# Ogeon/pyrite

Hardware: AMD Instinct MI355X
Metric: Msamples/sec (higher is better)
Workload: dtype f32; 1 GPU; C3: c3_mesh_in_box, 1920x1080, 1024 spp; bounces=8, light_samples=4, spectrum_samples=10, spectrum_bins=64, tile_size=32, triangles=819212, spheres=0, parallelism=one launch on one GPU, film_weight_check=ok

## Files before the change

### pyrite_amd/csrc/kernels.hip

```cpp
#ifndef PYRITE_KERNELS_HIP
#define PYRITE_KERNELS_HIP
#include <hip/hip_runtime.h>

#include <algorithm>
#include <cstdint>
#include <cstdlib>
#include <string>
#include <type_traits>

#include "device_scene.h"
#include "exact_math.h"

#ifdef PYR_WIDE_VM
#define PYR_VM_NUMBERS PYR_WIDE_NUMBER_REGISTERS
#define PYR_VM_VECTORS PYR_WIDE_VECTOR_REGISTERS
#define PYR_VM_RGBS PYR_WIDE_RGB_REGISTERS
#else
#define PYR_VM_NUMBERS PYR_MAX_NUMBER_REGISTERS
#define PYR_VM_VECTORS PYR_MAX_VECTOR_REGISTERS
#define PYR_VM_RGBS PYR_MAX_RGB_REGISTERS
#endif
static_assert((PYR_VM_NUMBERS & (PYR_VM_NUMBERS - 1)) == 0 && (PYR_VM_VECTORS & (PYR_VM_VECTORS - 1)) == 0 && (PYR_VM_RGBS & (PYR_VM_RGBS - 1)) == 0,
              "the interpreter masks register indices: its files are powers of two");

// ... 1153 lines not shown
            const float* from = reinterpret_cast<const float*>(src);
            if (COPY)
                for (uint32_t i = threadIdx.x; i < floats; i += BLOCK) dst[i] = from[i];
            float* at = dst;
            dst += floats;
            return at;
        };
        local.spectra = reinterpret_cast<const PyrSpectrum*>(stage(S.spectra, S.num_spectra * (uint32_t)(sizeof(PyrSpectrum) / sizeof(float))));
        local.spectrum_data = stage(S.spectrum_data, S.num_spectrum_floats);
        local.materials = reinterpret_cast<const PyrMaterial*>(stage(S.materials, S.num_materials * (uint32_t)(sizeof(PyrMaterial) / sizeof(float))));
        local.components = reinterpret_cast<const PyrComponent*>(stage(S.components, S.num_components * (uint32_t)(sizeof(PyrComponent) / sizeof(float))));
        local.programs = reinterpret_cast<const DevProgram*>(stage(S.programs, S.num_programs * (uint32_t)(sizeof(DevProgram) / sizeof(float))));
        local.lamps = reinterpret_cast<const DevLamp*>(stage(S.lamps, S.num_lamps * (uint32_t)(sizeof(DevLamp) / sizeof(float))));
        if (COPY) __syncthreads();
    }
    return local;
}

template <bool COMPANION_STATE = true>
DEV void start_sample(const RenderLaunch& L, uint32_t tile, uint64_t iteration, const TileArea& area, Path& p, Spectral& spec) {
    const uint32_t SS = L.spectrum_samples;
    p.rng = rng_seed(L.seed, tile, iteration);
    const float px = __fadd_rn(area.from_x, __fmul_rn(area.size_x, rng_f32(p.rng)));
    const float py = __fadd_rn(area.from_y, __fmul_rn(area.size_y, rng_f32(p.rng)));
    p.pixel = film_pixel(L, tile, px, py);
    {
        float focus_x = px / L.camera.view_plane * L.camera.focus_distance;
        float focus_y = py / L.camera.view_plane * L.camera.focus_distance;
        f3 target = mk(focus_x, -focus_y, -L.camera.focus_distance);
        f3 origin = mk(0, 0, 0), direction = target;
        if (L.camera.aperture > 0.0f) {
            float sqrt_r = sqrt32(L.camera.aperture * rng_f32(p.rng));
            float psi = PI_F * 2.0f * rng_f32(p.rng);
            origin = mk(sqrt_r * cos32(psi), sqrt_r * sin32(psi), 0.0f);
            direction = target - origin;
        }
        p.o = transform_point(L.camera.cam_to_world, origin);
        p.d = transform_vector(L.camera.cam_to_world, normalize(direction));
    }
    {
        float step_size = L.film.wl_width / (float)SS;
        float from = L.film.wl_start;
        for (uint32_t k = 0; k < SS; ++k) {
            float to = __fadd_rn(from, step_size);
            spec.wl(k) = rng_range_f32(p.rng, from, to);
            from = to;
        }
        uint32_t hero = rng_range_usize(p.rng, SS);
        p.wl = spec.wl(hero);
        spec.wl(hero) = spec.wl(SS - 1);
        if constexpr (COMPANION_STATE)
            for (uint32_t k = 0; k + 1 < SS; ++k) {
                spec.bright(k) = 0.0f;
                spec.refl(k) = 1.0f;
            }
    }
    p.bright = 0.0f;
    p.refl = 1.0f;
    p.use_additional = true;
    p.sample_light = true;
    p.events = 0;
    p.bounce = 0;
}

DEV bool locate_chunk(const RenderLaunch& L, uint32_t chunk, uint32_t lane, uint32_t& tile, uint64_t& iteration, TileArea& area) {
    const uint32_t k = chunk / L.chunks_per_tile, within = chunk - k * L.chunks_per_tile;
    tile = L.tile_begin + k * L.tile_stride;
    const uint32_t ty = tile / L.tiles_x, tx = tile - ty * L.tiles_x;
    const uint32_t sx = tx * L.tile_size, sy = ty * L.tile_size;
    const uint32_t w = min(L.film.width - sx, L.tile_size), h = min(L.film.height - sy, L.tile_size);
    const uint64_t area_px = (uint64_t)w * h, iterations = area_px * L.pixel_samples;
    iteration = (uint64_t)within * 64u + lane;
    if (iteration >= iterations) return false;
    iteration += area_px * L.sample_begin;
    area = to_view_area(sx, sy, w, h, L.film.width, L.film.height);
    return true;
}

struct SyncProf {
    unsigned long long section[8] = {0, 0, 0, 0, 0, 0, 0, 0}, last = 0;
};
#ifdef PYR_PHASE_PROFILE
__device__ unsigned long long g_phase_prof[16];
#define SLAP(sp, i)                                 \
    {                                               \
        const unsigned long long now_ = clock64();  \
        (sp).section[i] += now_ - (sp).last;        \
        (sp).last = now_;                           \
    }
#else
#define SLAP(sp, i)
#endif

constexpr int SYNC_PRIO_T = 3, SYNC_PRIO_N = 2, SYNC_PRIO_S = 1, SYNC_PRIO_E = 0;
#define SYNC_PRIO(x) __builtin_amdgcn_s_setprio(x)
template <bool COUNT>
DEV bool bounce_step(const DevScene& S, const RenderLaunch& L, const SceneView& view, Path& p, Spectral& spec, int* stack, Counters& cnt, SyncProf& sp) {
    const uint32_t n_add = L.spectrum_samples - 1;
    Hit hit;
    if (COUNT) cnt.extension_rays++;
    const f3 ray_o = p.o, ray_d = p.d;
    SYNC_PRIO(SYNC_PRIO_T);
    const bool found = traverse<COUNT, false>(S, view.nodes, view.prims, ray_o, ray_d, 0.0f, hit, stack, cnt);
    SYNC_PRIO(SYNC_PRIO_S);
    SLAP(sp, 1);
    if (!found) {
        uint32_t color = S.sky_program;
        if (p.sample_light) {
            for (uint32_t i = 0; i < S.num_lamps; ++i) {
                const DevLamp& l = S.lamps[i];
                if (l.kind == PYR_LAMP_DIRECTIONAL && dot(ld3(l.v), ray_d) >= l.width) {
                    color = l.color_program;
                    break;
                }
            }
        }
        const Prepared q_prog = prepare_program<false>(S, color);
        VmInput in{p.wl, -ray_d, ray_d};
        p.bright += eval_prepared<false>(S, q_prog, in) * 1.0f * p.refl;
        if (p.use_additional)
            for (uint32_t k = 0; k < n_add; ++k) {
                in.wavelength = spec.wl(k);
                spec.bright(k) += eval_prepared<false>(S, q_prog, in) * 1.0f * spec.refl(k);
            }
        return true;
    }
    if (COUNT) cnt.shaded_hits++;
    f3 position, normal;
    uint32_t material_id;
    surface_at(S, hit, ray_o, ray_d, position, normal, material_id);
    const PyrMaterial material = S.materials[material_id];
    const uint32_t pick = rng_choose(p.rng, material.num_components);
    const PyrComponent comp = S.components[material.first_component + pick];
    float component_probability = comp.selection_compensation;
    bool normal_dispersed = false;
    if (comp.probability_program >= 0) {
        VmInput pin{p.wl, normal, ray_d};
        component_probability = run_program<false>(S, (uint32_t)comp.probability_program, pin) * comp.selection_compensation;
        normal_dispersed = S.programs[comp.probability_program].reads_wavelength != 0;
    }

    if (comp.bsdf == PYR_BSDF_EMISSIVE) {
        if (p.sample_light) {
            p.use_additional = !normal_dispersed && p.use_additional;
            const Prepared q_prog = prepare_program<false>(S, comp.color_program);
            VmInput in{p.wl, normal, ray_d};
            p.bright += eval_prepared<false>(S, q_prog, in) * component_probability * p.refl;
            if (p.use_additional)
                for (uint32_t k = 0; k < n_add; ++k) {
                    in.wavelength = spec.wl(k);
                    spec.bright(k) += eval_prepared<false>(S, q_prog, in) * component_probability * spec.refl(k);
                }
        }
        return true;
    }

    f3 out_direction;
    float scatter_probability = 1.0f;
    bool dispersed = false, has_brdf = false;
    if (comp.bsdf == PYR_BSDF_DIFFUSE) {
        f3 n = dot(ray_d, normal) < 0.0f ? normal : -normal;
        out_direction = sample_hemisphere(p.rng, n);
        has_brdf = true;
    } else if (comp.bsdf == PYR_BSDF_MIRROR) {
        f3 n = dot(ray_d, normal) < 0.0f ? normal : -normal;
        float perp = dot(ray_d, n) * 2.0f;
// ... 112 lines not shown
        if (p.use_additional)
            for (uint32_t k = 0; k < n_add; ++k) spec.refl(k) *= brdf;
    }
    p.o = position;
    p.d = out_direction;
    SLAP(sp, 6);
    return false;
}

template <bool COUNT>
DEV void finish_path(const RenderLaunch& L, const Path& p, Spectral& spec, Counters& cnt) {
    expose_grain<COUNT>(L, p.pixel, p.wl, p.bright, cnt);
    if (p.use_additional)
        for (uint32_t k = 0; k + 1 < L.spectrum_samples; ++k) expose_grain<COUNT>(L, p.pixel, spec.wl(k), spec.bright(k), cnt);
}

typedef __attribute__((address_space(4))) const RenderLaunch* kernarg_launch_ptr;
constexpr size_t kLaunchKernargOffset = (sizeof(DevScene) + alignof(RenderLaunch) - 1) / alignof(RenderLaunch) * alignof(RenderLaunch);
typedef __attribute__((address_space(4))) const DevScene* kernarg_scene_ptr;
DEV const DevScene& scene_from_kernarg(const DevScene& ) {
    unsigned long long at = (unsigned long long)__builtin_amdgcn_kernarg_segment_ptr();
    asm volatile("" : "+s"(at));
    return *(const DevScene*)(kernarg_scene_ptr)at;
}
DEV const RenderLaunch& launch_from_kernarg(const RenderLaunch& ) {
    unsigned long long at = (unsigned long long)__builtin_amdgcn_kernarg_segment_ptr() + kLaunchKernargOffset;
    asm volatile("" : "+s"(at));
    return *(const RenderLaunch*)(kernarg_launch_ptr)at;
}

template <bool COUNT, bool LDS_SCENE, bool LDS_TABLES>
__global__ __launch_bounds__(BLOCK, 4) void render_kernel(DevScene S0, RenderLaunch L) {
    extern __shared__ float lds[];
    const uint32_t SS = L.spectrum_samples;
    Spectral spec{lds + threadIdx.x, SS};
    int* stack = reinterpret_cast<int*>(lds + 3 * SS * BLOCK) + threadIdx.x;
    Counters cnt{};
    const uint32_t lds_base_floats = (3 * SS + S0.stack_depth) * BLOCK;
    const SceneView view = stage_scene<LDS_SCENE>(S0, lds, lds_base_floats);
    const DevScene S = stage_tables<LDS_TABLES ? 1 : 0>(S0, lds, lds_base_floats + (LDS_SCENE ? (S0.num_nodes * 16 + S0.num_prims * 12) : 0));

    const uint32_t lane = threadIdx.x & 63u;
    const uint32_t waves_per_block = BLOCK / 64;
    const uint32_t wave = blockIdx.x * waves_per_block + (threadIdx.x >> 6);
    const uint32_t total_waves = gridDim.x * waves_per_block;

    SyncProf sp;
#ifdef PYR_PHASE_PROFILE
    sp.last = clock64();
#endif
    for (uint32_t chunk = L.chunk_begin + wave; chunk < L.chunk_end; chunk += total_waves) {
        uint32_t tile;
        uint64_t iteration;
        TileArea area;
        if (!locate_chunk(L, chunk, lane, tile, iteration, area)) continue;
        Path p{};
        start_sample(launch_from_kernarg(L), tile, iteration, area, p, spec);
        if (COUNT) cnt.samples++;
        SLAP(sp, 0);
        while (p.bounce < L.bounces) {
            const bool ended = bounce_step<COUNT>(S, launch_from_kernarg(L), view, p, spec, stack, cnt, sp);
            p.bounce++;
            if (ended) break;
        }
        SLAP(sp, 6);
        SYNC_PRIO(SYNC_PRIO_E);
        finish_path<COUNT>(launch_from_kernarg(L), p, spec, cnt);
        SLAP(sp, 7);
    }
#ifdef PYR_PHASE_PROFILE
    if (lane == 0)
        for (int i = 0; i < 8; ++i) atomicAdd(&g_phase_prof[i], sp.section[i]);
#endif
    flush_counters<COUNT>(cnt, L.counters);
}

#ifdef PYR_PHASE_PROFILE
#define PROF_DECL unsigned long long prof_c[4] = {0, 0, 0, 0}, prof_l[4] = {0, 0, 0, 0}, prof_n[4] = {0, 0, 0, 0}
#define PROF_BEGIN(ph, cond) const unsigned long long prof_t0_##ph = clock64(); prof_l[ph] += __popcll(ballot64(cond)); prof_n[ph]++
#define PROF_END(ph) prof_c[ph] += clock64() - prof_t0_##ph
#define PROF_LANES(ph, cond) prof_l[ph] += __popcll(ballot64(cond)); prof_n[ph]++
#define PROF_NOW() clock64()
#define PROF_EXTRA(idx, cycles) if ((threadIdx.x & 63u) == 0) atomicAdd(&g_phase_prof[idx], (unsigned long long)(cycles))
#define PROF_FLUSH()                                                                                  \
    if ((threadIdx.x & 63u) == 0)                                                                     \
        for (int i = 0; i < 4; ++i) {                                                                 \
            atomicAdd(&g_phase_prof[i], prof_c[i]);                                                   \
            atomicAdd(&g_phase_prof[4 + i], prof_l[i]);                                               \
            atomicAdd(&g_phase_prof[8 + i], prof_n[i]);                                               \
        }
#else
#define PROF_DECL
#define PROF_BEGIN(ph, cond)
#define PROF_END(ph)
#define PROF_LANES(ph, cond)
#define PROF_NOW() 0ull
#define PROF_EXTRA(idx, cycles)
#define PROF_FLUSH()
#endif

enum Stage : uint32_t { ST_NEW = 0, ST_TRAV = 1, ST_SHADE = 2, ST_NEE = 3, ST_EXPOSE = 4, ST_DONE = 5 };

struct Trav {
    f3 o, d, inv;
    uint32_t nx = 0, ny = 0, nz = 0;
    float limit, closest;
    int node, sp;
    uint32_t shape;
    float u, v;
    bool shadow, blocked;
};

DEV void trav_ray_signs(Trav& t) {
    t.nx = (__float_as_uint(t.d.x) >> 31) * 48u;
    t.ny = (__float_as_uint(t.d.y) >> 31) * 48u;
    t.nz = (__float_as_uint(t.d.z) >> 31) * 48u;
}
DEV float shadow_cutoff(float limit, float margin) { return __builtin_amdgcn_sqrtf(limit * margin + 1.0e-3f); }
DEV void trav_restart(Trav& t, float shadow_margin) {
    if (t.shadow) t.closest = shadow_cutoff(t.limit, shadow_margin);
    t.blocked = false;
    t.node = 0;
    t.sp = 0;
}

template <bool COUNT>
DEV bool trav_begin(const DevScene& S, Trav& t, f3 o, f3 d, bool shadow, float limit, Counters& cnt) {
    t.o = o;
    t.d = d;
    t.shadow = shadow;
    t.blocked = false;
    t.limit = shadow ? limit : -PYR_INF;
    t.closest = PYR_INF;
    t.shape = PYR_HIT_NONE;
    t.u = t.v = 0.0f;
    for (uint32_t i = 0; i < S.num_planes; ++i) {
        const float* pl = S.planes + 8 * i;
        float dist;
        f3 point;
        if (COUNT) cnt.plane_tests++;
        if (plane_test(ld3(pl), ld3(pl + 3), o, d, dist, point)) {
            if (shadow) {
                if (dist > DIST_EPSILON && dist * dist < limit) {
                    t.blocked = true;
                    return true;
                }
            } else if (dist > DIST_EPSILON && dist < t.closest) {
                t.closest = dist;
                t.shape = ((uint32_t)PYR_SHAPE_PLANE << 30) | i;
            }
        }
    }
    trav_restart(t, S.shadow_margin);
    return false;
}

typedef __attribute__((address_space(3))) int lds_int;
struct TravStack {
    lds_int* lds;
    int lds_entries;
    int* deep;
    DEV void push(int sp, int value) {
        if (sp < lds_entries)
            lds[sp * BLOCK] = value;
        else
            deep[sp - lds_entries] = value;
    }
    DEV int pop(int sp) const { return sp < lds_entries ? lds[sp * BLOCK] : deep[sp - lds_entries]; }
};

template <bool COUNT, bool SIGNED = false>
DEV void wide_node_children(const float4 lx, const float4 ly, const float4 lz, const float4 hx, const float4 hy, const float4 hz, const float4 ch, const Trav& t,
                            Counters& cnt, float (&e)[4], int (&c)[4]) {
    const f2v ix = {t.inv.x, t.inv.x}, iy = {t.inv.y, t.inv.y}, iz = {t.inv.z, t.inv.z};
    const float ox = -(t.o.x * t.inv.x), oy = -(t.o.y * t.inv.y), oz = -(t.o.z * t.inv.z);
    const f2v nox = {ox, ox}, noy = {oy, oy}, noz = {oz, oz};
    c[0] = __float_as_int(ch.x), c[1] = __float_as_int(ch.y), c[2] = __float_as_int(ch.z), c[3] = __float_as_int(ch.w);
    {
        const f2v alx = __builtin_elementwise_fma((f2v){lx.x, lx.y}, ix, nox), ahx = __builtin_elementwise_fma((f2v){hx.x, hx.y}, ix, nox);
        const f2v aly = __builtin_elementwise_fma((f2v){ly.x, ly.y}, iy, noy), ahy = __builtin_elementwise_fma((f2v){hy.x, hy.y}, iy, noy);
// ... 690 lines not shown
                    contribution(CONTRIB_ADD, l_color, deferred_probability, material_probability, true, ls_scale, p.use_additional && !l_dispersed, target_normal, t.d,
                                 ls_physical ? ls_tx : 0.0f, ls_physical ? ls_ty : 0.0f);
                } else {
                    const Prepared q_prog = prepare_program<INTERP>(S, l_color);
                    VmInput in{p.wl, target_normal, t.d, ls_physical ? ls_tx : 0.0f, ls_physical ? ls_ty : 0.0f};
                    p.bright += eval_prepared<INTERP>(S, q_prog, in) * l_probability * p.refl;
                    if (p.use_additional && !l_dispersed)
                        for (uint32_t k = 0; k < n_add; ++k) {
                            in.wavelength = spec.wl(k);
                            spec.bright(k) += eval_prepared<INTERP>(S, q_prog, in) * l_probability * spec.refl(k);
                        }
                }
            }
        }
        const DevLamp& lamp = S.lamps[nee_lamp];
        while (nee_i < L.light_samples) {
            const LampSample ls = lamp_sample<INTERP>(lamp, p.rng, b_position);
            nee_i++;
            const float cos_out = fmaxf(dot(b_nff(), ls.direction), 0.0f);
            if (!(cos_out > 0.0f)) continue;
            if (COUNT) cnt.shadow_rays++;
            const float limit = ls.sq_distance >= 0.0f ? ls.sq_distance - DIST_EPSILON : PYR_INF;
            ls_scale = ls.weight * nee_probability(S, L) * (2.0f * fabsf(dot(ls.direction, b_nff())));
            ls_physical = ls.physical;
            ls_material = ls.material;
            ls_color = ls.color;
            ls_normal = ls.normal;
            ls_tx = ls.tx, ls_ty = ls.ty;
            ls_pending = true;
            stage = trav_begin<COUNT>(S, t, b_position, ls.direction, true, limit, cnt) ? ST_NEE : ST_TRAV;
            break;
        }
        if (stage == ST_NEE && !ls_pending) finish_bounce(S, L, spec, cnt);
    }
};

DEV float lambda_eval(const DevScene& S, const DevProgram& p, float wavelength) {
    float num[PYR_MAX_NUMBER_REGISTERS];
    auto value = [&](const PyrOperand& o) -> float {
        if (o.kind == PYR_OPERAND_CONSTANT) return __uint_as_float(o.bits);
        if (o.kind == PYR_OPERAND_INPUT) return wavelength;
        return num[o.bits & (PYR_MAX_NUMBER_REGISTERS - 1)];
    };
    for (uint32_t k = 0; k < p.num_instrs; ++k) {
        const PyrInstr& ins = S.instrs[p.first_instr + k];
        float r = 0.0f;
        switch (ins.op) {
        case PYR_OP_NUMBER: r = __uint_as_float(ins.x.bits); break;
        case PYR_OP_SPECTRUM: r = spectrum_get(S, ins.a, value(ins.x)); break;
        case PYR_OP_BLACKBODY: {
            const float wl = value(ins.x), temp = value(ins.y);
            r = blackbody(wl, temp);
            break;
        }
        case PYR_OP_MIX: {
            const float amount = fmaxf(fminf(value(ins.x), 1.0f), 0.0f);
            const float l = num[ins.a & (PYR_MAX_NUMBER_REGISTERS - 1)], rr = num[ins.b & (PYR_MAX_NUMBER_REGISTERS - 1)];
            r = l * (1.0f - amount) + rr * amount;
            break;
        }
        case PYR_OP_BINARY: {
            const float l = num[ins.a & (PYR_MAX_NUMBER_REGISTERS - 1)], rr = num[ins.b & (PYR_MAX_NUMBER_REGISTERS - 1)];
            r = ins.operator_ == PYR_BIN_ADD ? l + rr : (ins.operator_ == PYR_BIN_SUB ? l - rr : (ins.operator_ == PYR_BIN_MUL ? l * rr : l / rr));
            break;
        }
        default: {
            const float v = value(ins.x), mn = value(ins.y), mx = value(ins.z);
            r = fmaxf(fminf(v, mx), mn);
            break;
        }
        }
        num[ins.output & (PYR_MAX_NUMBER_REGISTERS - 1)] = r;
    }
    return num[p.output_reg & (PYR_MAX_NUMBER_REGISTERS - 1)];
}

template <bool COUNT, bool RGB = false, bool TIMES = false>
DEV void replay_tapes(const DevScene& S, const RenderLaunch& L, bool exposing, uint32_t n_ops, uint32_t tape_column, const Path& p, const float* wl_rows,
                      uint32_t wl_column, uint32_t* wave_list, const uint32_t* prepared_lds, float* spectral_values, uint32_t n_spectral, bool eager, Counters& cnt) {
    const uint32_t lane = threadIdx.x & 63u;
    const unsigned long long mask = ballot64(exposing);
    const uint32_t n = (uint32_t)__popcll(mask);
    if (n == 0) return;
    uint32_t max_ops = exposing ? (n_ops < L.tape_max_ops ? n_ops : L.tape_max_ops) : 0u;
    const uint32_t my_ops = max_ops;
    for (int off = 32; off > 0; off >>= 1) max_ops = max(max_ops, (uint32_t)__shfl_xor((int)max_ops, off));
    const bool keeps = exposing && p.use_additional, lost = exposing && !p.use_additional;
    const bool longest = 3u * my_ops > 2u * max_ops, shortest = 3u * my_ops <= max_ops;
    const unsigned long long below = (1ull << lane) - 1ull;
    const unsigned long long k0 = ballot64(keeps && longest), k1 = ballot64(keeps && !longest && !shortest), k2 = ballot64(keeps && shortest);
    const unsigned long long l0 = ballot64(lost && longest), l1 = ballot64(lost && !longest && !shortest), l2 = ballot64(lost && shortest);
    const uint32_t n_full = (uint32_t)__builtin_popcountll(k0 | k1 | k2);
    if (exposing) {
        const unsigned long long mine = keeps ? (longest ? k0 : (shortest ? k2 : k1)) : (longest ? l0 : (shortest ? l2 : l1));
        uint32_t before = keeps ? 0u : n_full;
        before += (uint32_t)__builtin_popcountll(keeps ? ((longest ? 0ull : k0) | (shortest ? k1 : 0ull)) : ((longest ? 0ull : l0) | (shortest ? l1 : 0ull)));
        wave_list[before + (uint32_t)__builtin_popcountll(mine & below)] = lane;
    }
    __builtin_amdgcn_wave_barrier();
    const uint32_t SS = L.spectrum_samples, full_items = n_full * SS, items = full_items + (n - n_full);
    const unsigned long long past_the_end =
        eager ? ((unsigned long long)(kTapeOneSlot << TAPE_EAGER_SLOT_SHIFT) | ((unsigned long long)__float_as_uint(1.0f) << 32)) : 0ull;
#ifndef PYR_REPLAY_ROWS
#define PYR_REPLAY_ROWS 8
#endif
    constexpr uint32_t ROWS = PYR_REPLAY_ROWS;
    for (uint32_t base = 0; base < items; base += 64) {
        const uint32_t i = base + lane;
        const bool active = i < items;
        const bool full = i < full_items;
        const uint32_t rank = !active ? 0u : (full ? i / SS : n_full + (i - full_items)), k = !active ? 0u : (full ? i - rank * SS : SS - 1u);
        const uint32_t src = wave_list[rank];
        const uint32_t ops = (uint32_t)__shfl((int)n_ops, (int)src);
        uint32_t pass_ops = active ? (ops < L.tape_max_ops ? ops : L.tape_max_ops) : 0u;
        for (int off = 32; off > 0; off >>= 1) pass_ops = max(pass_ops, (uint32_t)__shfl_xor((int)pass_ops, off));
        const uint32_t pixel = (uint32_t)__shfl((int)p.pixel, (int)src);
        const float hero_wl = __shfl(p.wl, (int)src);
        const bool hero = k == SS - 1;
        const bool run = active;
        const uint32_t src_column = (uint32_t)__shfl((int)wl_column, (int)src);
        const float wl = hero ? hero_wl : wl_rows[k * BLOCK + src_column];
        float refl = 1.0f, bright = 0.0f, value = 0.0f;
        uint32_t value_of = 0xFFFFFFFFu;
        [[maybe_unused]] float rgb_sum = 0.0f;
        if (eager) {
            const uint32_t* slot_program = prepared_lds + 8 * L.tape_programs_lds;
            uint32_t grid_min = 0, grid_max = 0, grid_count = 0;
            uint32_t i0 = 0, i1 = 0;
            float mix = 0.0f;
            bool below = false, above = false;
            for (uint32_t slot = 0; slot < n_spectral; ++slot) {
                const uint32_t* e = prepared_lds + 8 * slot_program[slot];
                const uint32_t mode = e[0], format = e[2], count = e[6];
                const float c = __uint_as_float(e[1]);
                const float* data = S.spectrum_data + e[5];
                float v;
                if (RGB && mode == 0xFFu) {
                    v = lambda_eval(S, S.programs[slot_program[slot]], wl);
                } else if (format == PYR_SPECTRUM_ARRAY && count != 0u) {
                    if (e[3] != grid_min || e[4] != grid_max || count != grid_count) {
                        grid_min = e[3], grid_max = e[4], grid_count = count;
                        const float lo = __uint_as_float(grid_min), hi = __uint_as_float(grid_max);
                        below = wl <= lo, above = wl >= hi;
                        const float normalized = (wl - lo) / (hi - lo);
                        const float float_index = normalized * ((float)count - 1.0f);
                        const float min_float_index = truncf(float_index);
                        i0 = (below | above) ? 0u : (uint32_t)min_float_index;
                        i1 = (below | above) ? 0u : i0 + 1u;
                        mix = float_index - min_float_index;
                    }
                    const float inside = data[i0] * (1.0f - mix) + data[i1] * mix;
                    v = below ? data[0] : (above ? data[count - 1] : inside);
                } else {
                    PyrSpectrum sp;
                    sp.format = format, sp.min = __uint_as_float(e[3]), sp.max = __uint_as_float(e[4]), sp.offset = e[5], sp.count = count;
                    v = spectrum_eval(sp, data, wl);
                }
                spectral_values[tape_row(slot) * BLOCK] = (mode == FAST_SPECTRUM || mode == 0xFFu) ? v : v * c;
            }
            if (RGB && S.rgb_records != 0) {
                float resp[3] = {0.0f, 0.0f, 0.0f};
                const uint32_t count = S.rgb_count;
                if (count > 0) {
                    const float* d = S.rgb_basis;
                    if (wl <= S.rgb_min) {
                        for (int j = 0; j < 3; ++j) resp[j] = d[j];
                    } else if (wl >= S.rgb_max) {
                        for (int j = 0; j < 3; ++j) resp[j] = d[3 * (count - 1) + j];
                    } else {
                        const float normalized = (wl - S.rgb_min) / (S.rgb_max - S.rgb_min);
                        const float fi = normalized * ((float)count - 1.0f);
                        const float fmin_ = truncf(fi);
                        const uint32_t b0 = (uint32_t)fmin_;
                        const float bmix = fi - fmin_;
                        for (int j = 0; j < 3; ++j) resp[j] = d[3 * b0 + j] * (1.0f - bmix) + d[3 * (b0 + 1) + j] * bmix;
                    }
                }
                for (uint32_t j = 0; j < 3; ++j) spectral_values[(tape_rgb_row(n_spectral) + j) * BLOCK] = resp[j];
            }
        }
        for (uint32_t r0 = 0; r0 < pass_ops; r0 += ROWS) {
            unsigned long long rows[ROWS];
#pragma unroll
            for (uint32_t j = 0; j < ROWS; ++j) rows[j] = r0 + j < my_ops ? L.tape[tape_index(r0 + j, L.tape_lanes, tape_column)] : past_the_end;
            uint32_t words[ROWS];
            float factors[ROWS];
#pragma unroll
            for (uint32_t j = 0; j < ROWS; ++j) {
                words[j] = (uint32_t)__shfl((int)(uint32_t)rows[j], (int)src);
                factors[j] = __uint_as_float((uint32_t)__shfl((int)(uint32_t)(rows[j] >> 32), (int)src));
            }
            if (eager) {
                float values[ROWS];
#pragma unroll
                for (uint32_t j = 0; j < ROWS; ++j) values[j] = spectral_values[words[j] & TAPE_EAGER_SLOT_MASK];
                if (RGB && (TIMES ? S.micro_records : S.rgb_records) != 0) {
                    const uint32_t not_mine = hero ? 0u : TAPE_HERO_ONLY;
#pragma unroll
                    for (uint32_t j = 0; j < ROWS; ++j) {
                        const float m = values[j] * factors[j];
                        const uint32_t op = (words[j] >> TAPE_RGB_SHIFT) & (TIMES ? 7u : 3u);
                        if constexpr (TIMES)
                            rgb_sum = op == 1u ? m : (op == 2u ? rgb_sum + m : (op == 4u ? rgb_sum * m : rgb_sum));
                        else
                            rgb_sum = op == 1u ? m : (op == 2u ? rgb_sum + m : rgb_sum);
                        const float mm = op == 3u ? rgb_sum * factors[j] : m;
                        const bool apply = ((words[j] & not_mine) == 0u) & ((op == 0u) | (op == 3u));
                        const bool adds = (int)words[j] < 0;
                        const float multiplied = refl * mm, added = bright + multiplied;
                        bright = (apply & adds) ? added : bright;
                        refl = (apply & !adds) ? multiplied : refl;
                    }
                    continue;
                }
                if (S.hero_only_records == 0) {
#pragma unroll
                    for (uint32_t j = 0; j < ROWS; ++j) {
                        const float m = values[j] * factors[j];
                        const bool adds = (int)words[j] < 0;
                        const float multiplied = refl * m, added = bright + multiplied;
                        bright = adds ? added : bright;
                        refl = adds ? refl : multiplied;
                    }
                    continue;
                }
                const uint32_t not_for_me = hero ? 0u : TAPE_HERO_ONLY;
#pragma unroll
                for (uint32_t j = 0; j < ROWS; ++j) {
                    const float m = values[j] * factors[j];
                    const bool apply = (words[j] & not_for_me) == 0u;
                    const bool adds = (int)words[j] < 0;
                    const float multiplied = refl * m, added = bright + multiplied;
                    bright = (apply & adds) ? added : bright;
                    refl = (apply & !adds) ? multiplied : refl;
                }
                continue;
            }
#pragma unroll
            for (uint32_t j = 0; j < ROWS; ++j) {
                const uint32_t word = words[j];
                const float s = factors[j];
                if (!run || r0 + j >= ops) continue;
                const uint32_t kind = word >> 30;
                if (kind == TAPE_SCALE) {
                    refl *= s;
                    continue;
                }
                if ((word & TAPE_HERO_ONLY) && !hero) continue;
                const uint32_t program = word & TAPE_PROGRAM_MASK;
                if (program != value_of) {
                    Prepared q_prog;
                    if (program < L.tape_programs_lds) {
                        const uint32_t* e = prepared_lds + 8 * program;
                        q_prog.mode = e[0];
                        q_prog.c = __uint_as_float(e[1]);
                        q_prog.sp.format = e[2];
                        q_prog.sp.min = __uint_as_float(e[3]);
                        q_prog.sp.max = __uint_as_float(e[4]);
                        q_prog.sp.offset = e[5];
                        q_prog.sp.count = e[6];
                        q_prog.data = S.spectrum_data + e[5];
                        q_prog.id = program;
                    } else {
                        q_prog = prepare_program<false>(S, program);
                    }
                    VmInput in{wl, mk(0, 0, 0), mk(0, 0, 0)};
                    value = eval_prepared<false>(S, q_prog, in);
                    value_of = program;
                }
                if (kind == TAPE_MUL)
                    refl *= value * s;
                else
                    bright += value * s * refl;
            }
        }
        if (run) expose_grain<COUNT>(L, pixel, wl, bright, cnt);
    }
    __builtin_amdgcn_wave_barrier();
}

DEV uint32_t prepare_tape_tables(const DevScene& S0, const DevScene& S, const RenderLaunch& L, uint32_t* prepared_lds, bool& eager) {
    auto reads_spectrum = [&](uint32_t i) {
        return S0.programs[i].kind != PYR_PROGRAM_CONSTANT && (S0.programs[i].fast != FAST_NONE || (S0.hit_tape != 0 && S0.programs[i].tape_form == TAPE_FORM_LAMBDA));
    };
    auto alike = [&](uint32_t i, uint32_t j) {
        const DevProgram &a = S0.programs[i], &b = S0.programs[j];
        return a.fast != FAST_NONE && a.fast == b.fast && __float_as_uint(a.fast_scale) == __float_as_uint(b.fast_scale) && a.fast_spectrum == b.fast_spectrum;
    };
    auto first_alike = [&](uint32_t i) {
        for (uint32_t j = 0; j < i; ++j)
            if (reads_spectrum(j) && alike(i, j)) return j;
        return i;
    };
    auto slot_of = [&](uint32_t representative) {
        uint32_t slot = 0;
        for (uint32_t j = 0; j < representative; ++j) slot += (reads_spectrum(j) && first_alike(j) == j) ? 1u : 0u;
        return slot;
    };
    uint32_t n_spectral = 0;
    for (uint32_t i = 0; i < L.tape_programs_lds; ++i) n_spectral += (reads_spectrum(i) && first_alike(i) == i) ? 1u : 0u;
    for (uint32_t i = threadIdx.x; i < L.tape_programs_lds; i += BLOCK) {
        const Prepared q = prepare_program<false>(S, i);
        const bool spectral = reads_spectrum(i);
        const uint32_t representative = spectral ? first_alike(i) : i;
        const uint32_t slot = spectral ? slot_of(representative) : 0u;
        uint32_t* e = prepared_lds + 8 * i;
        e[0] = q.mode, e[1] = __float_as_uint(q.c), e[2] = q.sp.format, e[3] = __float_as_uint(q.sp.min), e[4] = __float_as_uint(q.sp.max);
        e[5] = q.sp.offset, e[6] = q.sp.count, e[7] = tape_row(slot);
        if (spectral && representative == i && slot < kTapeMaxValueRows - 1u) prepared_lds[8 * L.tape_programs_lds + slot] = i;
    }
    __syncthreads();
    eager = L.tape_programs_lds != 0 && tape_rows_needed(n_spectral, S0.rgb_records != 0) <= S0.tape_value_rows && (n_spectral != 0 || S0.hit_tape != 0);
    return eager ? n_spectral : 0u;
}

#ifndef PYR_SM_WAVES_INTERP
#define PYR_SM_WAVES_INTERP 3
#endif
constexpr int sm_waves(bool interp) { return interp ? PYR_SM_WAVES_INTERP : PYR_SM_WAVES; }
template <bool COUNT, bool INTERP, bool LDS_SCENE, bool LDS_TABLES, bool HIT_TAPE = false, bool PRODUCT = false>
__global__ __launch_bounds__(BLOCK, sm_waves(INTERP)) void render_kernel_sm(DevScene S0, RenderLaunch L) {
    extern __shared__ float lds[];
    static_assert(INTERP || !HIT_TAPE, "HIT_TAPE is a form of the interpreter build");
    static_assert(HIT_TAPE || !PRODUCT, "PRODUCT is a form of the hit tape (device_scene.h TapeForm)");
    constexpr bool TAPE = !INTERP || HIT_TAPE;
    const uint32_t SS = L.spectrum_samples;
    Spectral spec{lds + threadIdx.x, SS};
    const uint32_t spectral_rows = TAPE ? SS + 1 + S0.tape_value_rows : 3 * SS;
    TravStack stack;
    int deep_levels[LDS_SCENE ? 1 : kMaxStackDepth];
    stack.deep = deep_levels;
    stack.lds = (lds_int*)(reinterpret_cast<int*>(lds + spectral_rows * BLOCK) + threadIdx.x);
    stack.lds_entries = (int)L.stack_lds;
    Counters cnt{};
    const uint32_t lds_base_floats = (spectral_rows + L.stack_lds) * BLOCK;
    const SceneView view = stage_scene<LDS_SCENE>(S0, lds, lds_base_floats, true);
    const DevScene S = stage_tables<LDS_TABLES ? 1 : 0>(S0, lds, lds_base_floats + (LDS_SCENE ? (S0.num_nodes * 16 + S0.num_prims * 12) : 0));

    const uint32_t lane = threadIdx.x & 63u;
    const uint32_t waves_per_block = BLOCK / 64;
    const uint32_t total_waves = gridDim.x * waves_per_block;
    const int phase_lanes = (int)L.sm_phase_lanes, trav_steps = (int)L.sm_trav_steps;
    const int expose_lanes = TAPE ? (int)L.sm_expose_lanes : phase_lanes;
    Walker<COUNT, INTERP, TAPE, PRODUCT> w;
    w.chunk = L.chunk_begin + blockIdx.x * waves_per_block + (threadIdx.x >> 6);
    w.tape_prepared = nullptr;
    uint32_t* wave_list = reinterpret_cast<uint32_t*>(lds + SS * BLOCK) + (threadIdx.x & ~63u);
    uint32_t* prepared_lds = reinterpret_cast<uint32_t*>(lds + lds_base_floats + (LDS_SCENE ? (S0.num_nodes * 16 + S0.num_prims * 12) : 0) + (LDS_TABLES ? S0.lds_table_floats : 0));
    uint32_t n_spectral = 0;
    bool eager = false;
    float* spectral_values = lds + (SS + 1) * BLOCK + threadIdx.x;
    if constexpr (TAPE) {
        spectral_values[kTapeOneSlot * BLOCK] = 1.0f;
        n_spectral = prepare_tape_tables(S0, S, L, prepared_lds, eager);
        if (eager) w.tape_prepared = prepared_lds;
        w.rgb_slot = tape_rgb_row(n_spectral);
        w.tape_column = blockIdx.x * BLOCK + threadIdx.x;
        if (HIT_TAPE && !eager) *L.tape_overflow = 1u;
    }

    auto scene_view = [&](const RenderLaunch& Lp) {
        if (LDS_SCENE || INTERP) return S;
        const uint32_t rows = (TAPE ? Lp.spectrum_samples + 1 + S0.tape_value_rows : 3 * Lp.spectrum_samples) + Lp.stack_lds;
        return stage_tables<LDS_TABLES ? 1 : 0, false>(scene_from_kernarg(S0), lds, rows * BLOCK);
    };
    PROF_DECL;
    for (;;) {
        int nT = __popcll(ballot64(w.stage == ST_TRAV));
        int nS = __popcll(ballot64(w.stage == ST_SHADE));
        int nN = __popcll(ballot64(w.stage == ST_NEE));
        int nE = __popcll(ballot64(w.stage == ST_EXPOSE || w.stage == ST_NEW));
        if (max(max(nT, nS), max(nN, nE)) == 0) break;

        if (nE >= expose_lanes || nE == max(max(nT, nS), max(nN, nE))) {
            PHASE_PRIO(PYR_PRIO_E);
            PROF_BEGIN(0, w.stage == ST_EXPOSE || w.stage == ST_NEW);
            const RenderLaunch& Lp = launch_from_kernarg(L);
            const DevScene Sp = scene_view(Lp);
            if constexpr (TAPE)
                replay_tapes<COUNT, HIT_TAPE, PRODUCT>(Sp, Lp, w.stage == ST_EXPOSE, w.n_ops, w.tape_column, w.p, lds, threadIdx.x, wave_list, prepared_lds, spectral_values, n_spectral,
                                              HIT_TAPE ? eager : n_spectral != 0, cnt);
            w.expose_and_restart(Sp, Lp, spec, cnt, lane, total_waves);
            PROF_END(0);
            nT = __popcll(ballot64(w.stage == ST_TRAV));
            nS = __popcll(ballot64(w.stage == ST_SHADE));
            nE = 0;
        }
        if (nS >= phase_lanes || nS == max(max(nT, nS), max(nN, nE))) {
            PHASE_PRIO(PYR_PRIO_S);
            PROF_BEGIN(1, w.stage == ST_SHADE);
            const RenderLaunch& Lp = launch_from_kernarg(L);
            w.shade(scene_view(Lp), Lp, spec, cnt);
            PROF_END(1);
            nT = __popcll(ballot64(w.stage == ST_TRAV));
            nN = __popcll(ballot64(w.stage == ST_NEE));
            nE = __popcll(ballot64(w.stage == ST_EXPOSE || w.stage == ST_NEW));
            nS = 0;
        }
        if (nN >= phase_lanes || nN == max(max(nT, nS), max(nN, nE))) {
            PHASE_PRIO(PYR_PRIO_N);
            PROF_BEGIN(2, w.stage == ST_NEE);
            const RenderLaunch& Lp = launch_from_kernarg(L);
            w.next_event(scene_view(Lp), Lp, spec, cnt);
            PROF_END(2);
            nT = __popcll(ballot64(w.stage == ST_TRAV));
            nN = __popcll(ballot64(w.stage == ST_NEE));
            nE = __popcll(ballot64(w.stage == ST_EXPOSE || w.stage == ST_NEW));
        }
        if constexpr (INTERP) {
            const unsigned long long pending = ballot64(w.c_kind != 0u || w.c_has_scale);
            if (pending != 0ull) {
                [[maybe_unused]] const unsigned long long t_c0 = PROF_NOW();
                PROF_EXTRA(13, __popcll(pending));
                PROF_EXTRA(14, 1);
                const RenderLaunch& Lp = launch_from_kernarg(L);
                if constexpr (HIT_TAPE)
                    w.tape_pending(scene_view(Lp), Lp);
                else
                    w.contribute_pending(scene_view(Lp), Lp, spec);
                PROF_EXTRA(12, PROF_NOW() - t_c0);
            }
            w.contribution_clear();
        }
        if (nT >= phase_lanes || nT == max(max(nT, nS), max(nN, nE))) {
#ifdef PYR_PHASE_PROFILE
            const unsigned long long prof_t0_3 = clock64();
#endif
            PHASE_PRIO(PYR_PRIO_T);
            w.t.inv = box_reciprocal(w.t.d);
            trav_ray_signs(w.t);
            if (!LDS_SCENE && view.wide && view.pairs != nullptr) {
                for (int step = 0; step < trav_steps; ++step) {
                    PROF_LANES(3, w.stage == ST_TRAV);
                    if (trav_step_lean<COUNT>(view, w.t, stack, cnt, w.stage == ST_TRAV)) w.stage = w.t.shadow ? ST_NEE : ST_SHADE;
                }
            } else {
                for (int step = 0; step < trav_steps; ++step) {
                    PROF_LANES(3, w.stage == ST_TRAV);
                    if (trav_step_voted<COUNT, !LDS_SCENE>(view, w.t, stack, cnt, w.stage == ST_TRAV)) w.stage = w.t.shadow ? ST_NEE : ST_SHADE;
                }
            }
            PROF_END(3);
        }
    }
    PROF_FLUSH();
    flush_counters<COUNT>(cnt, L.counters);
}


struct WorkFeed {
    uint32_t next = 0, end = 0;
    uint32_t segment = 0, visited = 0;
    bool drained = false;
};
DEV uint32_t feed_segment_begin(uint32_t n, uint32_t segment) { return (uint32_t)(((uint64_t)n * segment / kFeedSegments) & ~63ull); }
DEV uint32_t feed_segment_end(uint32_t n, uint32_t segment) { return segment + 1 == kFeedSegments ? n : feed_segment_begin(n, segment + 1); }
DEV void feed_reserve(WorkFeed& f, uint32_t* cursors, uint32_t n, uint32_t reserve, uint32_t lane) {
    while (f.next == f.end && !f.drained) {
        const uint32_t begin = feed_segment_begin(n, f.segment), end = feed_segment_end(n, f.segment);
        uint32_t base = 0;
        if (lane == 0) base = atomicAdd(&cursors[f.segment * kFeedCursorStride], reserve);
        base = __shfl(base, 0, 64);
        if (base < end - begin) {
            f.next = begin + base;
            f.end = begin + min(base + reserve, end - begin);
// ... 88 lines not shown
```

### pyrite_amd/csrc/kernels/profile.hip

```cpp
#include "main.hip"
#include "interp.hip"
#include "product.hip"

namespace pyr {
RenderKernel pick_wide_kernel(bool, bool, bool) { return nullptr; }
}

extern "C" int pyr_debug_phase_profile(unsigned long long* out16, int reset) {
    if (hipDeviceSynchronize() != hipSuccess) return -1;
    if (hipMemcpyFromSymbol(out16, HIP_SYMBOL(pyr::g_phase_prof), 16 * sizeof(unsigned long long)) != hipSuccess) return -1;
    if (reset) {
        unsigned long long zero[16] = {};
        if (hipMemcpyToSymbol(HIP_SYMBOL(pyr::g_phase_prof), zero, sizeof(zero)) != hipSuccess) return -1;
    }
    return 0;
}
```

Measured before the change: 629.5 Msamples/s.

## Sort replay wave list by key and trim tape tail batches

Replaces the six-ballot bucket ordering of exposing lanes with a full rank sort by a packed key (keeps flag, op count, lane) computed through readlane comparisons. Pass op counts come from two readlanes over the sorted list instead of a per-pass shuffle reduction. In eager mode the final partial batch of tape rows is applied in 4- and 2-row chunks so padded rows are skipped. Replay profiling counters are added behind the profile flag. The sort loop costs up to 64 readlanes per call, and the tail path adds code size and register pressure.

```diff
diff --git a/pyrite_amd/csrc/kernels.hip b/pyrite_amd/csrc/kernels.hip
--- a/pyrite_amd/csrc/kernels.hip
+++ b/pyrite_amd/csrc/kernels.hip
@@ -1259,6 +1259,7 @@
 };
 #ifdef PYR_PHASE_PROFILE
 __device__ unsigned long long g_phase_prof[16];
+__device__ unsigned long long g_replay_prof[16];
 #define SLAP(sp, i)                                 \
     {                                               \
         const unsigned long long now_ = clock64();  \
@@ -1537,6 +1538,15 @@
 #define PROF_LANES(ph, cond) prof_l[ph] += __popcll(ballot64(cond)); prof_n[ph]++
 #define PROF_NOW() clock64()
 #define PROF_EXTRA(idx, cycles) if ((threadIdx.x & 63u) == 0) atomicAdd(&g_phase_prof[idx], (unsigned long long)(cycles))
+#define RPROF_T0(t) const unsigned long long t = clock64()
+#define RPROF_T1(idx, t) RPROF_ADD(idx, clock64() - t)
+#define RPROF_ADD(idx, v) if ((threadIdx.x & 63u) == 0) atomicAdd(&g_replay_prof[idx], (unsigned long long)(v))
+#define RPROF_SUM(idx, v)                                                                             \
+    {                                                                                                 \
+        uint32_t rprof_sum = (v);                                                                     \
+        for (int off = 32; off > 0; off >>= 1) rprof_sum += (uint32_t)__shfl_xor((int)rprof_sum, off); \
+        RPROF_ADD(idx, rprof_sum);                                                                    \
+    }
 #define PROF_FLUSH()                                                                                  \
     if ((threadIdx.x & 63u) == 0)                                                                     \
         for (int i = 0; i < 4; ++i) {                                                                 \
@@ -1551,6 +1561,10 @@
 #define PROF_LANES(ph, cond)
 #define PROF_NOW() 0ull
 #define PROF_EXTRA(idx, cycles)
+#define RPROF_T0(t)
+#define RPROF_T1(idx, t)
+#define RPROF_ADD(idx, v)
+#define RPROF_SUM(idx, v)
 #define PROF_FLUSH()
 #endif
 
@@ -2407,22 +2421,17 @@
     const unsigned long long mask = ballot64(exposing);
     const uint32_t n = (uint32_t)__popcll(mask);
     if (n == 0) return;
-    uint32_t max_ops = exposing ? (n_ops < L.tape_max_ops ? n_ops : L.tape_max_ops) : 0u;
-    const uint32_t my_ops = max_ops;
-    for (int off = 32; off > 0; off >>= 1) max_ops = max(max_ops, (uint32_t)__shfl_xor((int)max_ops, off));
-    const bool keeps = exposing && p.use_additional, lost = exposing && !p.use_additional;
-    const bool longest = 3u * my_ops > 2u * max_ops, shortest = 3u * my_ops <= max_ops;
-    const unsigned long long below = (1ull << lane) - 1ull;
-    const unsigned long long k0 = ballot64(keeps && longest), k1 = ballot64(keeps && !longest && !shortest), k2 = ballot64(keeps && shortest);
-    const unsigned long long l0 = ballot64(lost && longest), l1 = ballot64(lost && !longest && !shortest), l2 = ballot64(lost && shortest);
-    const uint32_t n_full = (uint32_t)__builtin_popcountll(k0 | k1 | k2);
-    if (exposing) {
-        const unsigned long long mine = keeps ? (longest ? k0 : (shortest ? k2 : k1)) : (longest ? l0 : (shortest ? l2 : l1));
-        uint32_t before = keeps ? 0u : n_full;
-        before += (uint32_t)__builtin_popcountll(keeps ? ((longest ? 0ull : k0) | (shortest ? k1 : 0ull)) : ((longest ? 0ull : l0) | (shortest ? l1 : 0ull)));
-        wave_list[before + (uint32_t)__builtin_popcountll(mine & below)] = lane;
-    }
+    RPROF_T0(t_list);
+    const uint32_t my_ops = exposing ? (n_ops < L.tape_max_ops ? n_ops : L.tape_max_ops) : 0u;
+    const bool keeps = exposing && p.use_additional;
+    const uint32_t n_full = (uint32_t)__popcll(ballot64(keeps));
+    const uint32_t key = (keeps ? 0x80000000u : 0u) | (my_ops << 6) | lane;
+    uint32_t before = 0;
+    for (unsigned long long rest = mask; rest != 0ull; rest &= rest - 1ull)
+        before += (uint32_t)__builtin_amdgcn_readlane((int)key, (int)__builtin_ctzll(rest)) > key ? 1u : 0u;
+    if (exposing) wave_list[before] = lane;
     __builtin_amdgcn_wave_barrier();
+    RPROF_T1(0, t_list);
     const uint32_t SS = L.spectrum_samples, full_items = n_full * SS, items = full_items + (n - n_full);
     const unsigned long long past_the_end =
         eager ? ((unsigned long long)(kTapeOneSlot << TAPE_EAGER_SLOT_SHIFT) | ((unsigned long long)__float_as_uint(1.0f) << 32)) : 0ull;
@@ -2437,8 +2446,14 @@
         const uint32_t rank = !active ? 0u : (full ? i / SS : n_full + (i - full_items)), k = !active ? 0u : (full ? i - rank * SS : SS - 1u);
         const uint32_t src = wave_list[rank];
         const uint32_t ops = (uint32_t)__shfl((int)n_ops, (int)src);
-        uint32_t pass_ops = active ? (ops < L.tape_max_ops ? ops : L.tape_max_ops) : 0u;
-        for (int off = 32; off > 0; off >>= 1) pass_ops = max(pass_ops, (uint32_t)__shfl_xor((int)pass_ops, off));
+        const uint32_t listed_ops = (uint32_t)__shfl((int)my_ops, (int)src);
+        const uint32_t first_lost = base < full_items && full_items - base < 64u && full_items < items ? full_items - base : 0u;
+        const uint32_t pass_ops =
+            max((uint32_t)__builtin_amdgcn_readfirstlane((int)listed_ops), (uint32_t)__builtin_amdgcn_readlane((int)listed_ops, (int)first_lost));
+        RPROF_ADD(5, 1);
+        RPROF_ADD(7, min(items - base, 64u));
+        RPROF_SUM(8, active ? listed_ops : 0u);
+        RPROF_T0(t_values);
         const uint32_t pixel = (uint32_t)__shfl((int)p.pixel, (int)src);
         const float hero_wl = __shfl(p.wl, (int)src);
         const bool hero = k == SS - 1;
@@ -2504,25 +2519,31 @@
                 for (uint32_t j = 0; j < 3; ++j) spectral_values[(tape_rgb_row(n_spectral) + j) * BLOCK] = resp[j];
             }
         }
-        for (uint32_t r0 = 0; r0 < pass_ops; r0 += ROWS) {
-            unsigned long long rows[ROWS];
+        RPROF_T1(1, t_values);
+        RPROF_T0(t_rows);
+        auto load = [&](uint32_t r0, unsigned long long* rows) {
 #pragma unroll
             for (uint32_t j = 0; j < ROWS; ++j) rows[j] = r0 + j < my_ops ? L.tape[tape_index(r0 + j, L.tape_lanes, tape_column)] : past_the_end;
-            uint32_t words[ROWS];
-            float factors[ROWS];
+        };
+        auto apply = [&](auto n_rows, auto lazy, uint32_t r0, const unsigned long long* rows) {
+            constexpr uint32_t N = decltype(n_rows)::value;
+            [[maybe_unused]] constexpr bool LAZY = decltype(lazy)::value;
+            RPROF_ADD(6, N);
+            uint32_t words[N];
+            float factors[N];
 #pragma unroll
-            for (uint32_t j = 0; j < ROWS; ++j) {
+            for (uint32_t j = 0; j < N; ++j) {
                 words[j] = (uint32_t)__shfl((int)(uint32_t)rows[j], (int)src);
                 factors[j] = __uint_as_float((uint32_t)__shfl((int)(uint32_t)(rows[j] >> 32), (int)src));
             }
             if (eager) {
-                float values[ROWS];
+                float values[N];
 #pragma unroll
-                for (uint32_t j = 0; j < ROWS; ++j) values[j] = spectral_values[words[j] & TAPE_EAGER_SLOT_MASK];
+                for (uint32_t j = 0; j < N; ++j) values[j] = spectral_values[words[j] & TAPE_EAGER_SLOT_MASK];
                 if (RGB && (TIMES ? S.micro_records : S.rgb_records) != 0) {
                     const uint32_t not_mine = hero ? 0u : TAPE_HERO_ONLY;
 #pragma unroll
-                    for (uint32_t j = 0; j < ROWS; ++j) {
+                    for (uint32_t j = 0; j < N; ++j) {
                         const float m = values[j] * factors[j];
                         const uint32_t op = (words[j] >> TAPE_RGB_SHIFT) & (TIMES ? 7u : 3u);
                         if constexpr (TIMES)
@@ -2536,22 +2557,22 @@
                         bright = (apply & adds) ? added : bright;
                         refl = (apply & !adds) ? multiplied : refl;
                     }
-                    continue;
+                    return;
                 }
                 if (S.hero_only_records == 0) {
 #pragma unroll
-                    for (uint32_t j = 0; j < ROWS; ++j) {
+                    for (uint32_t j = 0; j < N; ++j) {
                         const float m = values[j] * factors[j];
                         const bool adds = (int)words[j] < 0;
                         const float multiplied = refl * m, added = bright + multiplied;
                         bright = adds ? added : bright;
                         refl = adds ? refl : multiplied;
                     }
-                    continue;
+                    return;
                 }
                 const uint32_t not_for_me = hero ? 0u : TAPE_HERO_ONLY;
 #pragma unroll
-                for (uint32_t j = 0; j < ROWS; ++j) {
+                for (uint32_t j = 0; j < N; ++j) {
                     const float m = values[j] * factors[j];
                     const bool apply = (words[j] & not_for_me) == 0u;
                     const bool adds = (int)words[j] < 0;
@@ -2559,47 +2580,74 @@
                     bright = (apply & adds) ? added : bright;
                     refl = (apply & !adds) ? multiplied : refl;
                 }
-                continue;
-            }
+                return;
+            }
+            if constexpr (LAZY) {
 #pragma unroll
-            for (uint32_t j = 0; j < ROWS; ++j) {
-                const uint32_t word = words[j];
-                const float s = factors[j];
-                if (!run || r0 + j >= ops) continue;
-                const uint32_t kind = word >> 30;
-                if (kind == TAPE_SCALE) {
-                    refl *= s;
-                    continue;
+                for (uint32_t j = 0; j < N; ++j) {
+                    const uint32_t word = words[j];
+                    const float s = factors[j];
+                    if (!run || r0 + j >= ops) continue;
+                    const uint32_t kind = word >> 30;
+                    if (kind == TAPE_SCALE) {
+                        refl *= s;
+                        continue;
+                    }
+                    if ((word & TAPE_HERO_ONLY) && !hero) continue;
+                    const uint32_t program = word & TAPE_PROGRAM_MASK;
+                    if (program != value_of) {
+                        Prepared q_prog;
+                        if (program < L.tape_programs_lds) {
+                            const uint32_t* e = prepared_lds + 8 * program;
+                            q_prog.mode = e[0];
+                            q_prog.c = __uint_as_float(e[1]);
+                            q_prog.sp.format = e[2];
+                            q_prog.sp.min = __uint_as_float(e[3]);
+                            q_prog.sp.max = __uint_as_float(e[4]);
+                            q_prog.sp.offset = e[5];
+                            q_prog.sp.count = e[6];
+                            q_prog.data = S.spectrum_data + e[5];
+                            q_prog.id = program;
+                        } else {
+                            q_prog = prepare_program<false>(S, program);
+                        }
+                        VmInput in{wl, mk(0, 0, 0), mk(0, 0, 0)};
+                        value = eval_prepared<false>(S, q_prog, in);
+                        value_of = program;
+                    }
+                    if (kind == TAPE_MUL)
+                        refl *= value * s;
+                    else
+                        bright += value * s * refl;
                 }
-                if ((word & TAPE_HERO_ONLY) && !hero) continue;
-                const uint32_t program = word & TAPE_PROGRAM_MASK;
-                if (program != value_of) {
-                    Prepared q_prog;
-                    if (program < L.tape_programs_lds) {
-                        const uint32_t* e = prepared_lds + 8 * program;
-                        q_prog.mode = e[0];
-                        q_prog.c = __uint_as_float(e[1]);
-                        q_prog.sp.format = e[2];
-                        q_prog.sp.min = __uint_as_float(e[3]);
-                        q_prog.sp.max = __uint_as_float(e[4]);
-                        q_prog.sp.offset = e[5];
-                        q_prog.sp.count = e[6];
-                        q_prog.data = S.spectrum_data + e[5];
-                        q_prog.id = program;
-                    } else {
-                        q_prog = prepare_program<false>(S, program);
-                    }
-                    VmInput in{wl, mk(0, 0, 0), mk(0, 0, 0)};
-                    value = eval_prepared<false>(S, q_prog, in);
-                    value_of = program;
-                }
-                if (kind == TAPE_MUL)
-                    refl *= value * s;
-                else
-                    bright += value * s * refl;
-            }
-        }
+            }
+        };
+        static_assert(ROWS >= 8 && (ROWS & (ROWS - 1)) == 0, "the remainder batches assume whole batches of a power of two >= 8");
+        unsigned long long rows[ROWS];
+        uint32_t r0 = 0;
+#ifndef PYR_REPLAY_TAIL
+#define PYR_REPLAY_TAIL 2
+#endif
+        for (const uint32_t body_end = eager && PYR_REPLAY_TAIL ? pass_ops & ~(ROWS - 1u) : pass_ops; r0 < body_end; r0 += ROWS) {
+            load(r0, rows);
+            apply(std::integral_constant<uint32_t, ROWS>{}, std::true_type{}, r0, rows);
+        }
+        if (PYR_REPLAY_TAIL && eager && r0 < pass_ops) {
+            load(r0, rows);
+            uint32_t left = pass_ops - r0;
+            if (left > 4u) {
+                apply(std::integral_constant<uint32_t, 4>{}, std::false_type{}, r0, rows);
+#pragma unroll
+                for (uint32_t j = 0; j < 4; ++j) rows[j] = rows[4 + j];
+                left -= 4u;
+            }
+            apply(std::integral_constant<uint32_t, 2>{}, std::false_type{}, r0, rows);
+            if (left > 2u) apply(std::integral_constant<uint32_t, 2>{}, std::false_type{}, r0, rows + 2);
+        }
+        RPROF_T1(2, t_rows);
+        RPROF_T0(t_grain);
         if (run) expose_grain<COUNT>(L, pixel, wl, bright, cnt);
+        RPROF_T1(3, t_grain);
     }
     __builtin_amdgcn_wave_barrier();
 }
@@ -2705,7 +2753,9 @@
             if constexpr (TAPE)
                 replay_tapes<COUNT, HIT_TAPE, PRODUCT>(Sp, Lp, w.stage == ST_EXPOSE, w.n_ops, w.tape_column, w.p, lds, threadIdx.x, wave_list, prepared_lds, spectral_values, n_spectral,
                                               HIT_TAPE ? eager : n_spectral != 0, cnt);
+            RPROF_T0(t_restart);
             w.expose_and_restart(Sp, Lp, spec, cnt, lane, total_waves);
+            RPROF_T1(4, t_restart);
             PROF_END(0);
             nT = __popcll(ballot64(w.stage == ST_TRAV));
             nS = __popcll(ballot64(w.stage == ST_SHADE));
diff --git a/pyrite_amd/csrc/kernels/profile.hip b/pyrite_amd/csrc/kernels/profile.hip
--- a/pyrite_amd/csrc/kernels/profile.hip
+++ b/pyrite_amd/csrc/kernels/profile.hip
@@ -15,3 +15,13 @@
     }
     return 0;
 }
+
+extern "C" int pyr_debug_replay_profile(unsigned long long* out16, int reset) {
+    if (hipDeviceSynchronize() != hipSuccess) return -1;
+    if (hipMemcpyFromSymbol(out16, HIP_SYMBOL(pyr::g_replay_prof), 16 * sizeof(unsigned long long)) != hipSuccess) return -1;
+    if (reset) {
+        unsigned long long zero[16] = {};
+        if (hipMemcpyToSymbol(HIP_SYMBOL(pyr::g_replay_prof), zero, sizeof(zero)) != hipSuccess) return -1;
+    }
+    return 0;
+}
```

Result: no change. 627.0 Msamples/s (-0.4%).
